# vikasdimaniya/video-fingerprinting

Measured on AMD Instinct MI355X. Metric: 1080p frames/sec embed+detect, higher is better.
Workload: dtype f32

## Files before the change

### include/offmark_hip.h

```cpp
#ifndef OFFMARK_HIP_H
#define OFFMARK_HIP_H

#include <stddef.h>
#include <stdint.h>

#ifdef __cplusplus
extern "C" {
#endif

#define OFMK_ABI_VERSION 6

#define OFMK_OK            0
#define OFMK_E_ARG        -1
#define OFMK_E_WORKSPACE  -2
#define OFMK_E_HIP        -3

int ofmk_version(void);
const char *ofmk_last_error(void);

typedef struct ofmk_timing ofmk_timing;
typedef struct ofmk_opts {
    uint32_t flags;
    uint32_t xcds;
    ofmk_timing *timing;
} ofmk_opts;
#define OFMK_F_SEPARATE_DETECT 1u
#define OFMK_F_LINEAR_TILES 2u
#define OFMK_F_XCD_TILES 4u
#define OFMK_XCD_TILES_MIN_BYTES 1194393600ull
#define OFMK_F_PARTIAL_COUNTS 8u
size_t ofmk_workspace_bytes(int frames_in_flight, int H, int W);

int ofmk_embed_rgb8(const uint8_t *in, uint8_t *out, int n, int H, int W,
                    const uint8_t *wm, int n_wm, const int32_t *wm_row, double alpha,
                    int chunk_frames, void *workspace, size_t workspace_bytes, void *stream,
                    const ofmk_opts *opts);

int ofmk_detect_rgb8(const uint8_t *in, int n, int H, int W, int L, double alpha,
                     int32_t *counts, uint8_t *bits,
                     int chunk_frames, void *workspace, size_t workspace_bytes, void *stream,
                     const ofmk_opts *opts);

int ofmk_detect_soft_rgb8(const uint8_t *in, int n, int H, int W, int L, double alpha, long long *soft,
                          int chunk_frames, void *workspace, size_t workspace_bytes, void *stream,
                          const ofmk_opts *opts);

int ofmk_embed_detect_rgb8(const uint8_t *in, uint8_t *out, int n, int H, int W,
                           const uint8_t *wm, int n_wm, const int32_t *wm_row, double alpha,
                           int L, int32_t *counts, uint8_t *bits,
                           int chunk_frames, void *workspace, size_t workspace_bytes, void *stream,
                           const ofmk_opts *opts);

int ofmk_svd_embed_rgb8(const uint8_t *in, uint8_t *out, int n, int H, int W,
                        const uint8_t *wm, int n_wm, const int32_t *wm_row, const double *scales, int blk, void *stream,
                        const ofmk_opts *opts);
int ofmk_svd_detect_rgb8(const uint8_t *in, int n, int H, int W, int L, const double *scales, int blk,
                         int32_t *counts, uint8_t *bits, void *stream, const ofmk_opts *opts);
int ofmk_svd_embed_detect_rgb8(const uint8_t *in, uint8_t *out, int n, int H, int W,
                               const uint8_t *wm, int n_wm, const int32_t *wm_row, const double *scales, int blk,
                               int L, int32_t *counts, uint8_t *bits, void *stream, const ofmk_opts *opts);
int ofmk_svd_detect_soft_rgb8(const uint8_t *in, int n, int H, int W, int L, const double *scales, int blk,
                              long long *soft, void *stream, const ofmk_opts *opts);
int ofmk_svd_sync_scores_rgb8(const uint8_t *in, int n, int H, int W, const double *scales, int blk, long long *scores,
// ... 118 lines not shown
int ofmk_halve_rgb8(const uint8_t *in, int n, int h, int w, uint8_t *out, void *stream, const ofmk_opts *opts);

int ofmk_signature_rgb8(const uint8_t *in, int n, int h, int w, uint8_t *sig, void *stream, const ofmk_opts *opts);
int ofmk_signature_distances(const uint8_t *a, int m, const uint8_t *b, int N, int32_t *dist, void *stream, const ofmk_opts *opts);
int ofmk_align_residuals_rgb8(const uint8_t *lib, int N, const uint8_t *leak, int m, int h, int w, int H, int W, const int32_t *first,
                              int span, const ofmk_affine *geom, long long *res, void *stream, const ofmk_opts *opts);

int ofmk_payloads_from_counts(const int32_t *counts, int n, int L, int n_bits, const int32_t *perm,
                              uint8_t *payload, void *stream, const ofmk_opts *opts);
int ofmk_svd_count_tiles(int H, int W, int blk);
int ofmk_payloads_from_partial_counts(const int32_t *partials, int tiles, int n, int L, int n_bits, const int32_t *perm,
                                      uint8_t *payload, int32_t *counts, void *stream, const ofmk_opts *opts);

int ofmk_encode_yuv32f(float *yuv, int n, int H, int W,
                       const uint8_t *wm, int n_wm, const int32_t *wm_row, double alpha,
                       int chunk_frames, void *workspace, size_t workspace_bytes, void *stream,
                       const ofmk_opts *opts);
int ofmk_decode_yuv32f(const float *yuv, int n, int H, int W, int L, double alpha,
                       int32_t *counts, uint8_t *bits,
                       int chunk_frames, void *workspace, size_t workspace_bytes, void *stream,
                       const ofmk_opts *opts);

int ofmk_debug_planes(const void *frame, int src_is_yuv32f, int H, int W, double alpha,
                      const uint8_t *wm,
                      float *y_dc, double *lum_mask, double *tex_mask, double *step,
                      float *c21_pre, float *c21_post,
                      void *workspace, size_t workspace_bytes, void *stream, const ofmk_opts *opts);

int ofmk_stage_analyze_rgb8(const uint8_t *in, int n, int H, int W,
                            void *workspace, size_t workspace_bytes, void *stream, const ofmk_opts *opts);
int ofmk_stage_mark_rgb8(const uint8_t *in, uint8_t *out, int n, int H, int W,
                         const uint8_t *wm, double alpha, int fused,
                         void *workspace, size_t workspace_bytes, void *stream, const ofmk_opts *opts);

int ofmk_hbm_copy(const void *src, void *dst, size_t bytes, void *stream);
int ofmk_hbm_read(const void *src, size_t bytes, void *sink, void *stream);

int ofmk_probe_xcc(int32_t *xcc_of_workgroup, int n_workgroups, void *stream, const ofmk_opts *opts);

#define OFMK_TIMING_KINDS 7
int ofmk_timing_create(int max_launches, unsigned kind_mask, ofmk_timing **out);
int ofmk_timing_collect(ofmk_timing *t, double *ms_by_kind , int *launches_by_kind );
int ofmk_timing_durations(ofmk_timing *t, float *ms_per_launch, int *kind_per_launch , int cap);
void ofmk_timing_destroy(ofmk_timing *t);

#ifdef __cplusplus
}
#endif
#endif
```

### video-fingerprinting_amd/csrc/offmark_kernels.hip

```cpp
#include <hip/hip_runtime.h>
#include <hip/hip_ext.h>

#include <atomic>
#include <cstdint>
#include <cstdio>
#include <cstring>
#include <type_traits>

#include "../../include/offmark_hip.h"

#include "common.hiph"
#include "readout.hiph"
#include "dct_kernels.hiph"
#include "svd_kernels.hiph"
#include "svd8_kernels.hiph"
#include "misc_kernels.hiph"
#include "planar_kernels.hiph"
#include "svd_planar_kernels.hiph"
#include "copies_kernels.hiph"
#include "planar_copies_kernels.hiph"
#include "resync_kernels.hiph"
#include "dct_resync_kernels.hiph"
#include "planar_resync_kernels.hiph"
#include "warp_kernels.hiph"
// ... 123 lines not shown

constexpr size_t kFixedBytes = 4096;

size_t tiles_per_frame(int H, int W) { return ((size_t)(H / 8) * (W / 8) + kThreads - 1) / kThreads; }

size_t per_frame_bytes(int H, int W) {
    const size_t nblk = (size_t)(H / 8) * (W / 8);
    return nblk * (kRec + 1) * sizeof(float) + 2 * tiles_per_frame(H, W) * 8;
}

int carve(void *ws, size_t bytes, int H, int W, int want_frames, Workspace &out) {
    if (!ws) return fail(OFMK_E_ARG, "workspace is null%s");
    if ((uintptr_t)ws % 256) return fail(OFMK_E_ARG, "workspace must be 256-byte aligned%s");
    const size_t per = per_frame_bytes(H, W);
    if (bytes < per + kFixedBytes) return fail(OFMK_E_WORKSPACE, "workspace smaller than ofmk_workspace_bytes(1, H, W)%s");
    size_t cap = (bytes - kFixedBytes) / per;
    if (want_frames > 0 && (size_t)want_frames < cap) cap = want_frames;
    if (cap > (size_t)kMaxChunk) cap = kMaxChunk;
    const size_t nblk = (size_t)(H / 8) * (W / 8);
    char *p = static_cast<char *>(ws);
    out.frames = (int)cap;
    out.tiles = (int)tiles_per_frame(H, W);
    out.plane = cap * nblk;
    out.rec = reinterpret_cast<float *>(p);
    p += align256(out.plane * kRec * sizeof(float));
    out.delta = reinterpret_cast<float *>(p);
    p += align256(out.plane * sizeof(float));
    out.ysum = reinterpret_cast<unsigned long long *>(p);
    p += align256(cap * out.tiles * 8);
    out.ysum2 = reinterpret_cast<unsigned long long *>(p);
    return OFMK_OK;
}

int check_opts(const ofmk_opts *o) {
    if (o && ((o->flags & ~(uint32_t)(OFMK_F_SEPARATE_DETECT | OFMK_F_LINEAR_TILES | OFMK_F_XCD_TILES | OFMK_F_PARTIAL_COUNTS)) || o->xcds > 64u))
        return fail(OFMK_E_ARG, "ofmk_opts: unknown flag bits or xcds > 64%s");
    if (o && (o->flags & OFMK_F_LINEAR_TILES) && (o->flags & OFMK_F_XCD_TILES))
        return fail(OFMK_E_ARG, "ofmk_opts: OFMK_F_LINEAR_TILES and OFMK_F_XCD_TILES exclude each other%s");
    return OFMK_OK;
}

int check_dims(int n, int H, int W) {
    if (n <= 0) return fail(OFMK_E_ARG, "n must be positive%s");
    if (H < 8 || W < 8) return fail(OFMK_E_ARG, "H and W must be at least 8%s");
    if ((long long)H * W >= (1LL << 28)) return fail(OFMK_E_ARG, "frame too large (H*W must be < 2^28)%s");
    return OFMK_OK;
}

int check_embed_args(const void *in, const void *out, int n, int H, int W, const uint8_t *wm, int n_wm) {
    int rc = check_dims(n, H, W);
    if (rc) return rc;
    if (!in || !out || !wm) return fail(OFMK_E_ARG, "null frame or watermark pointer%s");
    if (n_wm < 1) return fail(OFMK_E_ARG, "n_wm must be >= 1%s");
    return OFMK_OK;
}

int check_detect_args(const void *in, int n, int H, int W, int L, const int32_t *counts, const uint8_t *bits) {
    int rc = check_dims(n, H, W);
    if (rc) return rc;
    if (!in) return fail(OFMK_E_ARG, "null frame pointer%s");
    if (L < 1) return fail(OFMK_E_ARG, "payload length L must be >= 1%s");
    if (!counts && !bits) return fail(OFMK_E_ARG, "both outputs (counts, bits) are null%s");
    return OFMK_OK;
}

int check_soft_args(const void *in, int n, int H, int W, int L, const long long *soft) {
    if (int rc = check_dims(n, H, W)) return rc;
    if (!in || !soft) return fail(OFMK_E_ARG, "null pointer%s");
    if (L < 1) return fail(OFMK_E_ARG, "payload length L must be >= 1%s");
    return OFMK_OK;
}

Geom make_geom(int H, int W, const Workspace &ws, int frames = 0, int xcds = 0) {
    Geom g;
    g.frames = frames;
    g.xcds = xcds;
    g.W = W;
    g.wb = W / 8;
// ... 46 lines not shown
    with_bool(aligned_rows(frames, W, src == SRC_RGB8 ? 1 : 4), [&](auto al) {
        constexpr bool AL = decltype(al)::value;
        if (src == SRC_RGB8) OFMK_TIMED_LAUNCH(timing, (analyze_kernel<SRC_RGB8, AL>), grid, dim3(kThreads), kAnalyzeLdsCap, s, frames, g, ws.rec, ws.ysum, zero_counts, L);
        else OFMK_TIMED_LAUNCH(timing, (analyze_kernel<SRC_YUV32F, AL>), grid, dim3(kThreads), 0, s, frames, g, ws.rec, ws.ysum, zero_counts, L);
    });
    HIP_TRY(hipGetLastError());
    return OFMK_OK;
}

int launch_finalize(FinArgs a, int n, const Ctx &cx) {
    const int per_wg = kThreads * kFinItems;
    const dim3 grid((unsigned)((a.N + per_wg - 1) / per_wg), (unsigned)n);
    ScopedTiming timing(KIND_FINALIZE, cx);
    with_bool(a.delta || a.soft || a.y_dc || a.lum || a.tex || a.step || a.c21_pre || a.c21_post, [&](auto full) {
        OFMK_TIMED_LAUNCH(timing, finalize_kernel<decltype(full)::value>, grid, dim3(kThreads), 0, cx.s, a);
    });
    HIP_TRY(hipGetLastError());
    return OFMK_OK;
}

MarkArgs mark_args(const Workspace &ws, int H, int W, const uint8_t *wm, int n_wm, const int32_t *wm_row, double alpha) {
    MarkArgs m;
    m.rec = ws.rec;
    m.ysum = ws.ysum;
    m.wm = wm;
    m.wm_row = wm_row;
    m.n_wm = n_wm;
    m.N = (int)((long long)H * W / 64);
    m.alpha = alpha;
    return m;
}

int launch_mark_rgb8(const uint8_t *in, uint8_t *out, int n, int H, int W, const uint8_t *wm, int n_wm, const int32_t *wm_row,
                     double alpha, const Workspace &ws, bool fused, const Ctx &cx) {
    hipStream_t s = cx.s;
    const int xc = tile_xcds(cx, (size_t)n * H * W * 3);
    const Geom g = make_geom(H, W, ws, n, xc);
    const dim3 grid = xcd_grid(g.nblk, n, xc);
    const MarkArgs m = mark_args(ws, H, W, wm, n_wm, wm_row, alpha);
    {
        ScopedTiming timing(fused ? KIND_MARK_FUSED : KIND_MARK, cx);
        with_bool(aligned_rows(in, W, 1) && aligned_rows(out, W, 1), [&](auto al) {
            constexpr bool AL = decltype(al)::value;
            if (fused) OFMK_TIMED_LAUNCH(timing, (mark_rgb8_kernel<AL, true>), grid, dim3(kThreads), 0, s, in, out, g, m, ws.rec, ws.ysum2);
            else if (xc > 1) OFMK_TIMED_LAUNCH(timing, (mark_rgb8_kernel<AL, false, true>), grid, dim3(kThreads), 0, s, in, out, g, m, ws.rec, ws.ysum2);
            else OFMK_TIMED_LAUNCH(timing, (mark_rgb8_kernel<AL, false>), grid, dim3(kThreads), 0, s, in, out, g, m, ws.rec, ws.ysum2);
        });
    }
    HIP_TRY(hipGetLastError());
    if (in != out && (H % 8 || W % 8)) {
        launch_copy_fringe(in, out, n, H, W, (H / 8) * 8, (W / 8) * 8, s);
        HIP_TRY(hipGetLastError());
    }
    return OFMK_OK;
}

struct RecView {
    const float *rec;
    const unsigned long long *ysum;
    size_t plane;
    int tiles;
};
RecView input_records(const Workspace &ws) { return {ws.rec, ws.ysum, ws.plane, ws.tiles}; }
RecView marked_records(const Workspace &ws) { return {ws.rec, ws.ysum2, ws.plane, ws.tiles}; }

FinArgs fin_base(const RecView &v, int H, int W, double alpha) {
    FinArgs a;
    memset(&a, 0, sizeof(a));
    a.rec = v.rec;
    a.plane = v.plane;
    a.ysum = v.ysum;
    a.tiles = v.tiles;
    a.nblk = (H / 8) * (W / 8);
    a.N = (int)((long long)H * W / 64);
    a.L = 1;
    a.n_wm = 1;
    a.alpha = alpha;
// ... 572 lines not shown
    HIP_TRY(launch_zero(soft, (size_t)copies * n * L * sizeof(long long), cx.s));
    const bool on = a.scales[1] > 0.f;
    if (blk == 4) return fused(a, on ? soft : nullptr);
    return launch_svd8_copies(out, frame_bytes, copies, n, H, W, wm_rows, a, [&](uint8_t *out_q, const SvdArgs &b) {
        if (int rc = single(out_q, b)) return rc;
        if (!on) return (int)OFMK_OK;
        const size_t q = (size_t)(out_q - out) / ((size_t)n * frame_bytes);
        SvdArgs bs = b;
        bs.counts = reinterpret_cast<int32_t *>(soft + q * n * L);
        bs.bits = nullptr;
        bs.partial = 0;
        return soft_of(out_q, bs);
    });
}

enum FrameKind { FRAMES_RGB8, FRAMES_YUV32F, FRAMES_YUV420 };
struct FrameFmt {
    FrameKind kind;
    int layout;
    int H, W;
    size_t frame_bytes;
};
FrameFmt rgb8_frames(int H, int W) { return {FRAMES_RGB8, 0, H, W, (size_t)H * W * 3}; }
FrameFmt yuv32f_frames(int H, int W) { return {FRAMES_YUV32F, 0, H, W, (size_t)H * W * 3 * sizeof(float)}; }
FrameFmt yuv420_frames(int layout, int H, int W) { return {FRAMES_YUV420, layout, H, W, (size_t)H * W * 3 / 2}; }

int analyze_frames(const FrameFmt &f, const uint8_t *frames, int n, const Workspace &ws, const Ctx &cx, int32_t *zero_counts = nullptr,
                   int L = 0) {
    if (f.kind == FRAMES_YUV420) return launch_analyze_yuv420(frames, f.layout, n, f.H, f.W, ws, cx, zero_counts, L);
    return launch_analyze(frames, f.kind == FRAMES_RGB8 ? SRC_RGB8 : SRC_YUV32F, n, f.H, f.W, ws, cx, zero_counts, L);
}

int mark_frames(const FrameFmt &f, const uint8_t *in, uint8_t *out, int n, const uint8_t *wm, int n_wm, const int32_t *wm_row,
                double alpha, const Workspace &ws, bool fused, const Ctx &cx) {
    if (f.kind == FRAMES_RGB8) return launch_mark_rgb8(in, out, n, f.H, f.W, wm, n_wm, wm_row, alpha, ws, fused, cx);
    if (f.kind == FRAMES_YUV420) return launch_mark_yuv420(in, out, f.layout, n, f.H, f.W, wm, n_wm, wm_row, alpha, ws, fused, cx);
    if (fused || in != out) return fail(OFMK_E_ARG, "internal: float32 frames are marked in place, without verify%s");
    return launch_mark_yuv32f(reinterpret_cast<float *>(out), n, f.H, f.W, wm, n_wm, wm_row, alpha, ws, cx);
}

int mark_copies(const FrameFmt &f, const uint8_t *in, uint8_t *out, int copies, int n, int f0, int cf, const uint8_t *wm, int n_wm,
                const int32_t *wm_rows, double alpha, const Workspace &ws, const Ctx &cx) {
    if (f.kind == FRAMES_RGB8) return launch_mark_copies_rgb8(in, out, copies, n, f0, cf, f.H, f.W, wm, n_wm, wm_rows, alpha, ws, cx);
    if (f.kind == FRAMES_YUV420)
        return launch_mark_copies_yuv420(in, out, f.layout, copies, n, f0, cf, f.H, f.W, wm, n_wm, wm_rows, alpha, ws, cx);
    return fail(OFMK_E_ARG, "internal: no copies kernel for float32 frames%s");
}

int mark_verify_copies(const FrameFmt &f, const uint8_t *in, uint8_t *out, int copies, int n, int f0, int cf, const uint8_t *wm,
                       int n_wm, const int32_t *wm_rows, double alpha, int L, int32_t *zero_counts, const CopiesWorkspace &ws,
                       const Ctx &cx) {
    CopyRecs v;
    v.rec = ws.rec;
    v.ysum = ws.ysum;
    v.plane = ws.plane;
    v.rec_stride = (size_t)ws.base.frames * (f.H / 8) * (f.W / 8);
    v.ysum_stride = (size_t)ws.base.frames * ws.base.tiles;
    v.zero_counts = zero_counts ? zero_counts + (size_t)f0 * L : nullptr;
    v.L = L;
    if (f.kind == FRAMES_RGB8)
        return launch_mark_verify_copies_rgb8(in, out, copies, n, f0, cf, f.H, f.W, wm, n_wm, wm_rows, alpha, L, v, ws.base, cx);
    if (f.kind == FRAMES_YUV420)
        return launch_mark_verify_copies_yuv420(in, out, f.layout, copies, n, f0, cf, f.H, f.W, wm, n_wm, wm_rows, alpha, L, v, ws.base, cx);
    return fail(OFMK_E_ARG, "internal: no copies kernel for float32 frames%s");
}

int read_out(const RecView &v, const FrameFmt &f, size_t row, int cf, int L, double alpha, int32_t *counts, uint8_t *bits,
             long long *soft, const Ctx &cx) {
    FinArgs a = fin_base(v, f.H, f.W, alpha);
    a.L = L;
    if (counts || bits) {
        a.counts = counts ? counts + row * L : nullptr;
        a.bits = bits ? bits + row * a.N : nullptr;
        if (int rc = launch_finalize(a, cf, cx)) return rc;
    }
    if (!soft) return OFMK_OK;
    a.counts = nullptr;
    a.bits = nullptr;
    a.soft = soft + row * L;
    return launch_finalize(a, cf, cx);
}

int embed_chunk(const FrameFmt &f, const uint8_t *in, uint8_t *out, int f0, int cf, const uint8_t *wm, int n_wm, const int32_t *wm_row,
                double alpha, const Workspace &ws, bool verify, const Ctx &cx, int32_t *zero_counts = nullptr, int L = 0) {
    const size_t fo = (size_t)f0 * f.frame_bytes;
    if (int rc = analyze_frames(f, in + fo, cf, ws, cx, zero_counts ? zero_counts + (size_t)f0 * L : nullptr, L)) return rc;
    return mark_frames(f, in + fo, out + fo, cf, wm, n_wm, wm_row ? wm_row + f0 : nullptr, alpha, ws, verify, cx);
}

int detect_chunk(const FrameFmt &f, const uint8_t *in, int f0, int cf, int L, double alpha, int32_t *counts, uint8_t *bits,
                 long long *soft, const Workspace &ws, const Ctx &cx) {
    if (int rc = analyze_frames(f, in + (size_t)f0 * f.frame_bytes, cf, ws, cx, counts ? counts + (size_t)f0 * L : nullptr, L)) return rc;
    return read_out(input_records(ws), f, (size_t)f0, cf, L, alpha, counts, bits, soft, cx);
}

int embed_frames(const FrameFmt &f, const uint8_t *in, uint8_t *out, int n, const uint8_t *wm, int n_wm, const int32_t *wm_row,
                 double alpha, int chunk_frames, void *workspace, size_t workspace_bytes, void *stream, const ofmk_opts *opts) {
    Workspace ws;
    if (int rc = carve(workspace, workspace_bytes, f.H, f.W, chunk_frames, ws)) return rc;
    const Ctx cx = make_ctx(stream, opts);
    return for_chunks(n, ws.frames, [&](int f0, int cf) { return embed_chunk(f, in, out, f0, cf, wm, n_wm, wm_row, alpha, ws, false, cx); });
}

int detect_frames(const FrameFmt &f, const uint8_t *in, int n, int L, double alpha, int32_t *counts, uint8_t *bits, long long *soft,
                  int chunk_frames, void *workspace, size_t workspace_bytes, void *stream, const ofmk_opts *opts) {
    Workspace ws;
    if (int rc = carve(workspace, workspace_bytes, f.H, f.W, chunk_frames, ws)) return rc;
    const Ctx cx = make_ctx(stream, opts);
    if (soft) HIP_TRY(launch_zero(soft, (size_t)n * L * sizeof(long long), cx.s));
    return for_chunks(n, ws.frames, [&](int f0, int cf) { return detect_chunk(f, in, f0, cf, L, alpha, counts, bits, soft, ws, cx); });
}

int embed_detect_frames(const FrameFmt &f, const uint8_t *in, uint8_t *out, int n, const uint8_t *wm, int n_wm, const int32_t *wm_row,
                        double alpha, int L, int32_t *counts, uint8_t *bits, int chunk_frames, void *workspace, size_t workspace_bytes,
                        void *stream, const ofmk_opts *opts) {
    Workspace ws;
    if (int rc = carve(workspace, workspace_bytes, f.H, f.W, chunk_frames, ws)) return rc;
    const Ctx cx = make_ctx(stream, opts);
    return for_chunks(n, ws.frames, [&](int f0, int cf) {
        if (!(cx.flags & OFMK_F_SEPARATE_DETECT)) {
            if (int rc = embed_chunk(f, in, out, f0, cf, wm, n_wm, wm_row, alpha, ws, true, cx, counts, L)) return rc;
            return read_out(marked_records(ws), f, (size_t)f0, cf, L, alpha, counts, bits, nullptr, cx);
        }
        if (int rc = embed_chunk(f, in, out, f0, cf, wm, n_wm, wm_row, alpha, ws, false, cx)) return rc;
        return detect_chunk(f, out, f0, cf, L, alpha, counts, bits, nullptr, ws, cx);
    });
}

int embed_copies_frames(const FrameFmt &f, const uint8_t *in, uint8_t *out, int copies, int n, const uint8_t *wm, int n_wm,
                        const int32_t *wm_rows, double alpha, int chunk_frames, void *workspace, size_t workspace_bytes, void *stream,
                        const ofmk_opts *opts) {
    Workspace ws;
    if (int rc = carve(workspace, workspace_bytes, f.H, f.W, chunk_frames, ws)) return rc;
    const Ctx cx = make_ctx(stream, opts);
    int rc = for_chunks(n, ws.frames, [&](int f0, int cf) {
        if (int rc = analyze_frames(f, in + (size_t)f0 * f.frame_bytes, cf, ws, cx)) return rc;
        return mark_copies(f, in, out, copies, n, f0, cf, wm, n_wm, wm_rows, alpha, ws, cx);
    });
    if (rc) return rc;
    return launch_copy_fringe_copies(in, out, copies, n, f.H, f.W, cx.s);
}

int embed_detect_copies_frames(const FrameFmt &f, const uint8_t *in, uint8_t *out, int copies, int n, const uint8_t *wm, int n_wm,
                               const int32_t *wm_rows, double alpha, int L, int32_t *counts, uint8_t *bits, long long *soft,
                               int chunk_frames, void *workspace, size_t workspace_bytes, void *stream, const ofmk_opts *opts) {
    CopiesWorkspace ws;
    if (int rc = carve_copies(workspace, workspace_bytes, copies, f.H, f.W, chunk_frames, ws)) return rc;
    const Ctx cx = make_ctx(stream, opts);
    const bool hard = counts || bits;
    const int nblk = (f.H / 8) * (f.W / 8);
    const size_t N = (size_t)((long long)f.H * f.W / 64);
    if (soft) HIP_TRY(launch_zero(soft, (size_t)copies * n * L * sizeof(long long), cx.s));
    int rc = for_chunks(n, ws.base.frames, [&](int f0, int cf) {
        if (int rc = analyze_frames(f, in + (size_t)f0 * f.frame_bytes, cf, ws.base, cx)) return rc;
        if (!(cx.flags & OFMK_F_SEPARATE_DETECT)) {
// ... 363 lines not shown
    a.wm = wm;
    a.y_dc = y_dc;
    a.lum = lum_mask;
    a.tex = tex_mask;
    a.step = step;
    a.c21_pre = c21_pre;
    a.c21_post = wm ? c21_post : nullptr;
    return launch_finalize(a, 1, cx);
}

int ofmk_stage_analyze_rgb8(const uint8_t *in, int n, int H, int W, void *workspace, size_t workspace_bytes,
                            void *stream, const ofmk_opts *opts) {
    if (int orc = check_opts(opts)) return orc;
    int rc = check_dims(n, H, W);
    if (rc) return rc;
    if (!in) return fail(OFMK_E_ARG, "null frame pointer%s");
    Workspace ws;
    if ((rc = carve(workspace, workspace_bytes, H, W, n, ws))) return rc;
    if (ws.frames < n) return fail(OFMK_E_WORKSPACE, "stage call needs workspace for all n frames%s");
    return analyze_frames(rgb8_frames(H, W), in, n, ws, make_ctx(stream, opts));
}

int ofmk_stage_mark_rgb8(const uint8_t *in, uint8_t *out, int n, int H, int W, const uint8_t *wm, double alpha,
                         int fused, void *workspace, size_t workspace_bytes, void *stream, const ofmk_opts *opts) {
    if (int orc = check_opts(opts)) return orc;
    int rc = check_embed_args(in, out, n, H, W, wm, 1);
    if (rc) return rc;
    Workspace ws;
    if ((rc = carve(workspace, workspace_bytes, H, W, n, ws))) return rc;
    if (ws.frames < n) return fail(OFMK_E_WORKSPACE, "stage call needs workspace for all n frames%s");
    return mark_frames(rgb8_frames(H, W), in, out, n, wm, 1, nullptr, alpha, ws, fused != 0, make_ctx(stream, opts));
}

int ofmk_svd_embed_rgb8(const uint8_t *in, uint8_t *out, int n, int H, int W, const uint8_t *wm, int n_wm,
                        const int32_t *wm_row, const double *scales, int blk, void *stream, const ofmk_opts *opts) {
    if (int orc = check_opts(opts)) return orc;
    int rc = check_embed_args(in, out, n, H, W, wm, n_wm);
    if (rc) return rc;
    if ((rc = check_blk(blk))) return rc;
    SvdArgs a;
    if ((rc = make_svd_args(a, H, W, scales, false, wm, n_wm, wm_row, 1, nullptr, nullptr, nullptr))) return rc;
    return launch_svd_rgb8(in, out, n, H, W, SVD_EMBED, blk, a, make_ctx(stream, opts));
}

int ofmk_svd_detect_rgb8(const uint8_t *in, int n, int H, int W, int L, const double *scales, int blk, int32_t *counts, uint8_t *bits,
                         void *stream, const ofmk_opts *opts) {
    if (int orc = check_opts(opts)) return orc;
    int rc = check_detect_args(in, n, H, W, L, counts, bits);
    if (rc) return rc;
    if ((rc = check_blk(blk))) return rc;
    SvdArgs a;
    if ((rc = make_svd_args(a, H, W, scales, true, nullptr, 0, nullptr, L, counts, bits, opts))) return rc;
    if (!(a.scales[1] > 0.f)) return zero_svd_readout(n, H, W, blk, a, static_cast<hipStream_t>(stream));
    return launch_svd_rgb8(in, nullptr, n, H, W, SVD_DETECT, blk, a, make_ctx(stream, opts));
}

int ofmk_svd_detect_soft_rgb8(const uint8_t *in, int n, int H, int W, int L, const double *scales, int blk, long long *soft,
                              void *stream, const ofmk_opts *opts) {
    if (int orc = check_opts(opts)) return orc;
    int rc = check_soft_args(in, n, H, W, L, soft);
    if (rc) return rc;
    if ((rc = check_blk(blk))) return rc;
    return svd_detect_soft(n, H, W, L, scales, soft, stream, [&](const SvdArgs &a) {
        return launch_svd_rgb8(in, nullptr, n, H, W, SVD_DETECT_SOFT, blk, a, make_ctx(stream, opts));
    });
}
// ... 890 lines not shown
```

### video-fingerprinting_amd/offmark/_hip.py

```python
from __future__ import annotations

import ctypes as C
import os

_LIB_PATH = os.path.join(os.path.dirname(os.path.abspath(__file__)), "_lib", "liboffmark_hip.so")

ABI_VERSION = 6


class Opts(C.Structure):
    _fields_ = [("flags", C.c_uint32), ("xcds", C.c_uint32), ("timing", C.c_void_p)]
    _timing = None


F_SEPARATE_DETECT = 1
F_LINEAR_TILES = 2
F_XCD_TILES = 4
F_PARTIAL_COUNTS = 8
XCD_TILES_MIN_BYTES = 192 * 1080 * 1920 * 3
YUV_I420, YUV_NV12 = 0, 1
TIMING_KINDS = ("analyze", "finalize", "mark", "mark_fused", "svd", "planar_analyze", "planar_mark")

_vp, _i32, _f64, _sz, _u32 = C.c_void_p, C.c_int, C.c_double, C.c_size_t, C.c_uint
_op = C.POINTER(Opts)
_dp = C.POINTER(C.c_double)


class Warp(C.Structure):
    _fields_ = [("ay", C.c_int64), ("by", C.c_int64), ("ax", C.c_int64), ("bx", C.c_int64)]


_wp = C.POINTER(Warp)


class Affine(C.Structure):
    _fields_ = [("ayy", C.c_int64), ("ayx", C.c_int64), ("by", C.c_int64), ("axy", C.c_int64), ("axx", C.c_int64), ("bx", C.c_int64)]


_ap = C.POINTER(Affine)

SIGNATURES = {
    "ofmk_version": (_i32, []),
    "ofmk_last_error": (C.c_char_p, []),
    "ofmk_workspace_bytes": (_sz, [_i32, _i32, _i32]),
    "ofmk_embed_rgb8": (_i32, [_vp, _vp, _i32, _i32, _i32, _vp, _i32, _vp, _f64, _i32, _vp, _sz, _vp, _op]),
    "ofmk_detect_rgb8": (_i32, [_vp, _i32, _i32, _i32, _i32, _f64, _vp, _vp, _i32, _vp, _sz, _vp, _op]),
    "ofmk_detect_soft_rgb8": (_i32, [_vp, _i32, _i32, _i32, _i32, _f64, _vp, _i32, _vp, _sz, _vp, _op]),
    "ofmk_embed_detect_rgb8": (_i32, [_vp, _vp, _i32, _i32, _i32, _vp, _i32, _vp, _f64, _i32, _vp, _vp, _i32, _vp, _sz,
                                      _vp, _op]),
    "ofmk_encode_yuv32f": (_i32, [_vp, _i32, _i32, _i32, _vp, _i32, _vp, _f64, _i32, _vp, _sz, _vp, _op]),
    "ofmk_decode_yuv32f": (_i32, [_vp, _i32, _i32, _i32, _i32, _f64, _vp, _vp, _i32, _vp, _sz, _vp, _op]),
    "ofmk_debug_planes": (_i32, [_vp, _i32, _i32, _i32, _f64, _vp, _vp, _vp, _vp, _vp, _vp, _vp, _vp, _sz, _vp, _op]),
    "ofmk_stage_analyze_rgb8": (_i32, [_vp, _i32, _i32, _i32, _vp, _sz, _vp, _op]),
    "ofmk_stage_mark_rgb8": (_i32, [_vp, _vp, _i32, _i32, _i32, _vp, _f64, _i32, _vp, _sz, _vp, _op]),
    "ofmk_svd_embed_rgb8": (_i32, [_vp, _vp, _i32, _i32, _i32, _vp, _i32, _vp, _dp, _i32, _vp, _op]),
    "ofmk_svd_detect_rgb8": (_i32, [_vp, _i32, _i32, _i32, _i32, _dp, _i32, _vp, _vp, _vp, _op]),
    "ofmk_svd_detect_soft_rgb8": (_i32, [_vp, _i32, _i32, _i32, _i32, _dp, _i32, _vp, _vp, _op]),
    "ofmk_svd_sync_scores_rgb8": (_i32, [_vp, _i32, _i32, _i32, _dp, _i32, _vp, _vp, _op]),
    "ofmk_svd_detect_soft_window_rgb8": (_i32, [_vp, _i32, _i32, _i32, _i32, _i32, _i32, _i32, _i32, _dp, _i32, _vp, _vp, _op]),
    "ofmk_sync_workspace_bytes": (_sz, [_i32, _i32, _i32]),
    "ofmk_sync_scores_rgb8": (_i32, [_vp, _i32, _i32, _i32, _f64, _vp, _i32, _vp, _sz, _vp, _op]),
    "ofmk_detect_soft_window_rgb8": (_i32, [_vp, _i32, _i32, _i32, _i32, _i32, _i32, _i32, _i32, _f64, _vp, _i32, _vp, _sz, _vp, _op]),
    "ofmk_svd_embed_detect_rgb8": (_i32, [_vp, _vp, _i32, _i32, _i32, _vp, _i32, _vp, _dp, _i32, _i32, _vp, _vp, _vp, _op]),
    "ofmk_embed_copies_rgb8": (_i32, [_vp, _vp, _i32, _i32, _i32, _i32, _vp, _i32, _vp, _f64, _i32, _vp, _sz, _vp, _op]),
    "ofmk_svd_embed_copies_rgb8": (_i32, [_vp, _vp, _i32, _i32, _i32, _i32, _vp, _i32, _vp, _dp, _i32, _i32, _vp, _vp, _vp,
                                          _op]),
    "ofmk_copies_workspace_bytes": (_sz, [_i32, _i32, _i32, _i32]),
    "ofmk_embed_detect_copies_rgb8": (_i32, [_vp, _vp, _i32, _i32, _i32, _i32, _vp, _i32, _vp, _f64, _i32, _vp, _vp, _i32, _vp, _sz,
                                             _vp, _op]),
    "ofmk_embed_detect_copies_soft_rgb8": (_i32, [_vp, _vp, _i32, _i32, _i32, _i32, _vp, _i32, _vp, _f64, _i32, _vp, _vp, _vp, _i32, _vp,
                                                  _sz, _vp, _op]),
    "ofmk_svd_embed_copies_soft_rgb8": (_i32, [_vp, _vp, _i32, _i32, _i32, _i32, _vp, _i32, _vp, _dp, _i32, _i32, _vp, _vp, _vp, _vp,
                                               _op]),
    "ofmk_svd_encode_yuv32f": (_i32, [_vp, _i32, _i32, _i32, _vp, _i32, _vp, _dp, _i32, _vp, _op]),
    "ofmk_svd_decode_yuv32f": (_i32, [_vp, _i32, _i32, _i32, _dp, _i32, _vp, _vp, _op]),
    "ofmk_payloads_from_counts": (_i32, [_vp, _i32, _i32, _i32, _vp, _vp, _vp, _op]),
    "ofmk_svd_count_tiles": (_i32, [_i32, _i32, _i32]),
    "ofmk_payloads_from_partial_counts": (_i32, [_vp, _i32, _i32, _i32, _i32, _vp, _vp, _vp, _vp, _op]),
    "ofmk_embed_yuv420": (_i32, [_vp, _vp, _i32, _i32, _i32, _i32, _vp, _i32, _vp, _f64, _i32, _vp, _sz, _vp, _op]),
    "ofmk_detect_yuv420": (_i32, [_vp, _i32, _i32, _i32, _i32, _i32, _f64, _vp, _vp, _i32, _vp, _sz, _vp, _op]),
    "ofmk_detect_soft_yuv420": (_i32, [_vp, _i32, _i32, _i32, _i32, _i32, _f64, _vp, _i32, _vp, _sz, _vp, _op]),
    "ofmk_embed_detect_yuv420": (_i32, [_vp, _vp, _i32, _i32, _i32, _i32, _vp, _i32, _vp, _f64, _i32, _vp, _vp, _i32, _vp,
                                        _sz, _vp, _op]),
    "ofmk_svd_embed_yuv420": (_i32, [_vp, _vp, _i32, _i32, _i32, _i32, _vp, _i32, _vp, _dp, _i32, _vp, _op]),
    "ofmk_svd_detect_yuv420": (_i32, [_vp, _i32, _i32, _i32, _i32, _i32, _dp, _i32, _vp, _vp, _vp, _op]),
    "ofmk_svd_detect_soft_yuv420": (_i32, [_vp, _i32, _i32, _i32, _i32, _i32, _dp, _i32, _vp, _vp, _op]),
    "ofmk_svd_embed_detect_yuv420": (_i32, [_vp, _vp, _i32, _i32, _i32, _i32, _vp, _i32, _vp, _dp, _i32, _i32, _vp, _vp, _vp,
# ... 154 lines not shown
```

Before: 282,500.

## Compute readout bits in fused mark kernel and count from per-wave masks

The fused mark kernel now computes each block's readout bit and a 'settled' flag, then stores them as per-wave ballot masks in the spare delta workspace. A new readout kernel counts bits from these masks, so the finalize pass no longer has to reread the full three-plane record array for every block. Blocks that are not settled (too close to the decision threshold) presumably fall back to the exact computation. This costs extra work and register pressure in the mark kernel, and it only applies when counts are requested, no bits are requested, and L is a power of two up to 64.

```diff
diff --git a/include/offmark_hip.h b/include/offmark_hip.h
--- a/include/offmark_hip.h
+++ b/include/offmark_hip.h
@@ -29,6 +29,7 @@
 #define OFMK_F_XCD_TILES 4u
 #define OFMK_XCD_TILES_MIN_BYTES 1194393600ull
 #define OFMK_F_PARTIAL_COUNTS 8u
+#define OFMK_F_PLAIN_READOUT 16u
 size_t ofmk_workspace_bytes(int frames_in_flight, int H, int W);
 
 int ofmk_embed_rgb8(const uint8_t *in, uint8_t *out, int n, int H, int W,
@@ -213,6 +214,12 @@
 int ofmk_stage_mark_rgb8(const uint8_t *in, uint8_t *out, int n, int H, int W,
                          const uint8_t *wm, double alpha, int fused,
                          void *workspace, size_t workspace_bytes, void *stream, const ofmk_opts *opts);
+int ofmk_stage_mark_masks_rgb8(const uint8_t *in, uint8_t *out, int n, int H, int W,
+                               const uint8_t *wm, double alpha, double delta,
+                               void *workspace, size_t workspace_bytes, void *stream, const ofmk_opts *opts);
+int ofmk_stage_readout_masks_rgb8(int n, int H, int W, int L, double alpha, double delta,
+                                  int32_t *counts, int32_t *stats,
+                                  void *workspace, size_t workspace_bytes, void *stream, const ofmk_opts *opts);
 
 int ofmk_hbm_copy(const void *src, void *dst, size_t bytes, void *stream);
 int ofmk_hbm_read(const void *src, size_t bytes, void *sink, void *stream);
diff --git a/video-fingerprinting_amd/csrc/dct_finalize_body.inc b/video-fingerprinting_amd/csrc/dct_finalize_body.inc
--- /dev/null
+++ b/video-fingerprinting_amd/csrc/dct_finalize_body.inc
@@ -0,0 +1,55 @@
+    __shared__ int hist[kHistMax];
+    __shared__ FrameLum s_lum;
+    const int t = threadIdx.x;
+    const int f = blockIdx.y;
+    const int c0 = tile_x * (kThreads * kFinItems) + t;
+    const bool use_hist = (p.counts != nullptr || (FULL && p.soft != nullptr)) && p.L <= kHistMax;
+    const bool pow2 = (p.L & (p.L - 1)) == 0;
+    if (use_hist)
+        for (int k = t; k < p.L; k += kThreads) hist[k] = 0;
+    float a00[kFinItems], tcode[kFinItems], c21[kFinItems];
+#pragma unroll
+    for (int i = 0; i < kFinItems; ++i) {
+        const int c = c0 + i * kThreads;
+        const float *r = p.rec + (size_t)f * p.nblk + (c < p.nblk ? c : p.nblk - 1);
+        a00[i] = r[0]; tcode[i] = r[p.plane]; c21[i] = r[2 * p.plane];
+    }
+    frame_lum_to_lds(p.ysum, f, p.tiles, p.nblk, &s_lum);
+    __syncthreads();
+    const FrameLum fl = s_lum;
+    const FastLum fq = make_fast_lum(fl, p.alpha);
+    const bool by_ballot = !FULL && p.counts != nullptr && pow2 && p.L <= 64;
+    unsigned long long own_mask = 0;
+    if (by_ballot)
+        for (int j = (int)(t & 63) & (p.L - 1); j < 64; j += p.L) own_mask |= 1ull << j;
+    unsigned own = 0;
+#pragma unroll
+    for (int i = 0; i < kFinItems; ++i) {
+        const int c = c0 + i * kThreads;
+        int bit = 0;
+        if constexpr (FULL) {
+            if (c < p.nblk) finalize_block<FULL>(p, f, c, fl, use_hist, hist, a00[i], tcode[i], c21[i], bit);
+        } else if (c < p.nblk) {
+            bit = readout_bit_fast(a00[i], tcode[i], c21[i], fl, fq, p.alpha);
+            if (p.bits) p.bits[(size_t)f * p.N + c] = (uint8_t)bit;
+        }
+        if (c >= p.nblk && c < p.N && p.bits) p.bits[(size_t)f * p.N + c] = 0;
+        if (by_ballot) {
+            const unsigned long long hit = __ballot(bit != 0) & own_mask;
+            own += __popc((unsigned)hit) + __popc((unsigned)(hit >> 32));
+        } else if (p.counts) {
+            count_bit(p, f, c, bit, pow2, use_hist, hist);
+        }
+    }
+    if (by_ballot && (int)(t & 63) < p.L && own) {
+        if (use_hist) atomicAdd(&hist[t & (p.L - 1)], (int)own);
+        else atomicAdd(&p.counts[(size_t)f * p.L + (t & (p.L - 1))], (int)own);
+    }
+    if (use_hist) {
+        __syncthreads();
+        for (int k = t; k < p.L; k += kThreads) {
+            const int v = hist[k];
+            if (FULL && v && p.soft) atomicAdd(reinterpret_cast<unsigned long long *>(&p.soft[(size_t)f * p.L + k]), (unsigned long long)(long long)v);
+            else if (v) atomicAdd(&p.counts[(size_t)f * p.L + k], v);
+        }
+    }
diff --git a/video-fingerprinting_amd/csrc/dct_mark_rgb8_body.inc b/video-fingerprinting_amd/csrc/dct_mark_rgb8_body.inc
--- /dev/null
+++ b/video-fingerprinting_amd/csrc/dct_mark_rgb8_body.inc
@@ -0,0 +1,40 @@
+    __shared__ FrameLum s_lum;
+    __shared__ long long s_part[kThreads / 64];
+    const int tiles = tiles_of(g.nblk);
+    int f, bx;
+    if (!xcd_tile(g.xcds, tiles, g.frames, f, bx)) return;
+    const int c = bx * kThreads + threadIdx.x;
+    const bool valid = c < g.nblk;
+    const int cc = valid ? c : g.nblk - 1;
+    int bi, bj;
+    divmod_small(cc, g.wb, g.inv_wb, bi, bj);
+    const size_t off = (size_t)f * g.frame_stride + ((size_t)bi * 8 * g.W + (size_t)bj * 8) * 3;
+    const int pitch = g.W * 3;
+    Px8 raw[8];
+#pragma unroll
+    for (int r = 0; r < 8; ++r) raw[r] = load_px8<ALIGNED>(in + off + (size_t)r * pitch);
+#pragma unroll
+    for (int r = 0; r < 8; ++r) forget(raw[r]);
+    frame_lum_to_lds(m.ysum, f, tiles, g.nblk, &s_lum);
+    __syncthreads();
+    if (!FUSED && !valid) return;
+    float R[8][8], u1[4];
+    float d;
+    {
+        const float *r = m.rec + (size_t)f * g.nblk + cc;
+        const int row = wm_row_of(m.wm_row, f, m.n_wm);
+        d = mark_delta(r[0], r[g.plane], r[2 * g.plane], s_lum, m.alpha, m.wm[(size_t)row * m.N + cc]);
+    }
+    mark_rows<ALIGNED, FUSED, HOLD>(raw, d, valid, out + off, pitch, R, u1);
+    if constexpr (FUSED) {
+        const BlockFeat ft = block_features(R, u1);
+        if constexpr (MASKS) {
+            const FrameLum fl = s_lum;
+            const SettledBit sb = readout_bit_settled(ft.a00, ft.tex, ft.c21, fl, make_fast_lum(fl, m.alpha), delta);
+            WaveMasks wmk;
+            wmk.settled = __ballot(!valid || sb.settled);
+            wmk.bits = __ballot(valid && sb.bit != 0);
+            if ((threadIdx.x & 63) == 0) summary[((size_t)f * tiles + bx) * kWavesPerTile + (threadIdx.x >> 6)] = wmk;
+        }
+        emit_block(ft, valid, f, c, bx, tiles, g, rec_out, ysum_out, s_part);
+    }
diff --git a/video-fingerprinting_amd/csrc/offmark_kernels.hip b/video-fingerprinting_amd/csrc/offmark_kernels.hip
--- a/video-fingerprinting_amd/csrc/offmark_kernels.hip
+++ b/video-fingerprinting_amd/csrc/offmark_kernels.hip
@@ -179,8 +179,13 @@
     return OFMK_OK;
 }
 
+WaveMasks *masks_of(const Workspace &ws) { return reinterpret_cast<WaveMasks *>(ws.delta); }
+bool masks_fit(const Workspace &ws, int frames) {
+    return (size_t)frames * ws.tiles * kWavesPerTile * sizeof(WaveMasks) <= align256(ws.plane * sizeof(float));
+}
+
 int check_opts(const ofmk_opts *o) {
-    if (o && ((o->flags & ~(uint32_t)(OFMK_F_SEPARATE_DETECT | OFMK_F_LINEAR_TILES | OFMK_F_XCD_TILES | OFMK_F_PARTIAL_COUNTS)) || o->xcds > 64u))
+    if (o && ((o->flags & ~(uint32_t)(OFMK_F_SEPARATE_DETECT | OFMK_F_LINEAR_TILES | OFMK_F_XCD_TILES | OFMK_F_PARTIAL_COUNTS | OFMK_F_PLAIN_READOUT)) || o->xcds > 64u))
         return fail(OFMK_E_ARG, "ofmk_opts: unknown flag bits or xcds > 64%s");
     if (o && (o->flags & OFMK_F_LINEAR_TILES) && (o->flags & OFMK_F_XCD_TILES))
         return fail(OFMK_E_ARG, "ofmk_opts: OFMK_F_LINEAR_TILES and OFMK_F_XCD_TILES exclude each other%s");
@@ -191,6 +196,11 @@
     if (n <= 0) return fail(OFMK_E_ARG, "n must be positive%s");
     if (H < 8 || W < 8) return fail(OFMK_E_ARG, "H and W must be at least 8%s");
     if ((long long)H * W >= (1LL << 28)) return fail(OFMK_E_ARG, "frame too large (H*W must be < 2^28)%s");
+    return OFMK_OK;
+}
+
+int check_delta(double delta) {
+    if (!(delta >= 0.0) || !(delta <= 255.0)) return fail(OFMK_E_ARG, "delta must lie in [0, 255]%s");
     return OFMK_OK;
 }
 
@@ -303,7 +313,7 @@
 }
 
 int launch_mark_rgb8(const uint8_t *in, uint8_t *out, int n, int H, int W, const uint8_t *wm, int n_wm, const int32_t *wm_row,
-                     double alpha, const Workspace &ws, bool fused, const Ctx &cx) {
+                     double alpha, const Workspace &ws, bool fused, const Ctx &cx, bool masks = false, double delta = kReadoutDelta) {
     hipStream_t s = cx.s;
     const int xc = tile_xcds(cx, (size_t)n * H * W * 3);
     const Geom g = make_geom(H, W, ws, n, xc);
@@ -313,7 +323,8 @@
         ScopedTiming timing(fused ? KIND_MARK_FUSED : KIND_MARK, cx);
         with_bool(aligned_rows(in, W, 1) && aligned_rows(out, W, 1), [&](auto al) {
             constexpr bool AL = decltype(al)::value;
-            if (fused) OFMK_TIMED_LAUNCH(timing, (mark_rgb8_kernel<AL, true>), grid, dim3(kThreads), 0, s, in, out, g, m, ws.rec, ws.ysum2);
+            if (fused && masks) OFMK_TIMED_LAUNCH(timing, (mark_masks_rgb8_kernel<AL>), grid, dim3(kThreads), 0, s, in, out, g, m, ws.rec, ws.ysum2, masks_of(ws), delta);
+            else if (fused) OFMK_TIMED_LAUNCH(timing, (mark_rgb8_kernel<AL, true>), grid, dim3(kThreads), 0, s, in, out, g, m, ws.rec, ws.ysum2);
             else if (xc > 1) OFMK_TIMED_LAUNCH(timing, (mark_rgb8_kernel<AL, false, true>), grid, dim3(kThreads), 0, s, in, out, g, m, ws.rec, ws.ysum2);
             else OFMK_TIMED_LAUNCH(timing, (mark_rgb8_kernel<AL, false>), grid, dim3(kThreads), 0, s, in, out, g, m, ws.rec, ws.ysum2);
         });
@@ -952,8 +963,9 @@
 }
 
 int mark_frames(const FrameFmt &f, const uint8_t *in, uint8_t *out, int n, const uint8_t *wm, int n_wm, const int32_t *wm_row,
-                double alpha, const Workspace &ws, bool fused, const Ctx &cx) {
-    if (f.kind == FRAMES_RGB8) return launch_mark_rgb8(in, out, n, f.H, f.W, wm, n_wm, wm_row, alpha, ws, fused, cx);
+                double alpha, const Workspace &ws, bool fused, const Ctx &cx, bool masks = false) {
+    if (f.kind == FRAMES_RGB8) return launch_mark_rgb8(in, out, n, f.H, f.W, wm, n_wm, wm_row, alpha, ws, fused, cx, masks);
+    if (masks) return fail(OFMK_E_ARG, "internal: only the fused RGB8 mark kernel leaves read-out masks%s");
     if (f.kind == FRAMES_YUV420) return launch_mark_yuv420(in, out, f.layout, n, f.H, f.W, wm, n_wm, wm_row, alpha, ws, fused, cx);
     if (fused || in != out) return fail(OFMK_E_ARG, "internal: float32 frames are marked in place, without verify%s");
     return launch_mark_yuv32f(reinterpret_cast<float *>(out), n, f.H, f.W, wm, n_wm, wm_row, alpha, ws, cx);
@@ -986,9 +998,22 @@
 }
 
 int read_out(const RecView &v, const FrameFmt &f, size_t row, int cf, int L, double alpha, int32_t *counts, uint8_t *bits,
-             long long *soft, const Ctx &cx) {
+             long long *soft, const Ctx &cx, const MaskArgs *masks = nullptr) {
     FinArgs a = fin_base(v, f.H, f.W, alpha);
     a.L = L;
+    if (masks) {
+        if (!counts || bits || soft) return fail(OFMK_E_ARG, "internal: the read-out by masks gives counts only%s");
+        a.counts = counts + row * L;
+        const int fin_tiles = (a.N + kThreads * kFinItems - 1) / (kThreads * kFinItems);
+        const int mask_wgs = (a.tiles * kWavesPerTile + kThreads - 1) / kThreads;
+        const int spare = 1536 / cf > 1 ? 1536 / cf : 1;
+        const int per_frame = mask_wgs > (spare < fin_tiles ? spare : fin_tiles) ? mask_wgs : (spare < fin_tiles ? spare : fin_tiles);
+        const dim3 grid((unsigned)per_frame, (unsigned)cf);
+        ScopedTiming timing(KIND_FINALIZE, cx);
+        OFMK_TIMED_LAUNCH(timing, readout_masks_kernel, grid, dim3(kThreads), 0, cx.s, a, *masks);
+        HIP_TRY(hipGetLastError());
+        return OFMK_OK;
+    }
     if (counts || bits) {
         a.counts = counts ? counts + row * L : nullptr;
         a.bits = bits ? bits + row * a.N : nullptr;
@@ -1001,11 +1026,21 @@
     return launch_finalize(a, cf, cx);
 }
 
+bool masks_usable(const FrameFmt &f, int cf, int L, double alpha, const int32_t *counts, const uint8_t *bits, const Workspace &ws,
+                  const Ctx &cx) {
+    return f.kind == FRAMES_RGB8 && counts && !bits && L <= 64 && (L & (L - 1)) == 0 && alpha >= 1e-3 && alpha <= 1e6 &&
+           !(cx.flags & OFMK_F_PLAIN_READOUT) && masks_fit(ws, cf);
+}
+MaskArgs marked_masks(const Workspace &ws, double delta = kReadoutDelta, int32_t *stats = nullptr) {
+    return {masks_of(ws), ws.ysum, delta, stats};
+}
+
 int embed_chunk(const FrameFmt &f, const uint8_t *in, uint8_t *out, int f0, int cf, const uint8_t *wm, int n_wm, const int32_t *wm_row,
-                double alpha, const Workspace &ws, bool verify, const Ctx &cx, int32_t *zero_counts = nullptr, int L = 0) {
+                double alpha, const Workspace &ws, bool verify, const Ctx &cx, int32_t *zero_counts = nullptr, int L = 0,
+                bool masks = false) {
     const size_t fo = (size_t)f0 * f.frame_bytes;
     if (int rc = analyze_frames(f, in + fo, cf, ws, cx, zero_counts ? zero_counts + (size_t)f0 * L : nullptr, L)) return rc;
-    return mark_frames(f, in + fo, out + fo, cf, wm, n_wm, wm_row ? wm_row + f0 : nullptr, alpha, ws, verify, cx);
+    return mark_frames(f, in + fo, out + fo, cf, wm, n_wm, wm_row ? wm_row + f0 : nullptr, alpha, ws, verify, cx, masks);
 }
 
 int detect_chunk(const FrameFmt &f, const uint8_t *in, int f0, int cf, int L, double alpha, int32_t *counts, uint8_t *bits,
@@ -1039,8 +1074,10 @@
     const Ctx cx = make_ctx(stream, opts);
     return for_chunks(n, ws.frames, [&](int f0, int cf) {
         if (!(cx.flags & OFMK_F_SEPARATE_DETECT)) {
-            if (int rc = embed_chunk(f, in, out, f0, cf, wm, n_wm, wm_row, alpha, ws, true, cx, counts, L)) return rc;
-            return read_out(marked_records(ws), f, (size_t)f0, cf, L, alpha, counts, bits, nullptr, cx);
+            const bool masks = masks_usable(f, cf, L, alpha, counts, bits, ws, cx);
+            if (int rc = embed_chunk(f, in, out, f0, cf, wm, n_wm, wm_row, alpha, ws, true, cx, counts, L, masks)) return rc;
+            const MaskArgs ma = marked_masks(ws);
+            return read_out(marked_records(ws), f, (size_t)f0, cf, L, alpha, counts, bits, nullptr, cx, masks ? &ma : nullptr);
         }
         if (int rc = embed_chunk(f, in, out, f0, cf, wm, n_wm, wm_row, alpha, ws, false, cx)) return rc;
         return detect_chunk(f, out, f0, cf, L, alpha, counts, bits, nullptr, ws, cx);
@@ -1470,6 +1507,39 @@
     return mark_frames(rgb8_frames(H, W), in, out, n, wm, 1, nullptr, alpha, ws, fused != 0, make_ctx(stream, opts));
 }
 
+int ofmk_stage_mark_masks_rgb8(const uint8_t *in, uint8_t *out, int n, int H, int W, const uint8_t *wm, double alpha, double delta,
+                               void *workspace, size_t workspace_bytes, void *stream, const ofmk_opts *opts) {
+    if (int orc = check_opts(opts)) return orc;
+    int rc = check_embed_args(in, out, n, H, W, wm, 1);
+    if (rc) return rc;
+    if ((rc = check_delta(delta))) return rc;
+    Workspace ws;
+    if ((rc = carve(workspace, workspace_bytes, H, W, n, ws))) return rc;
+    if (ws.frames < n) return fail(OFMK_E_WORKSPACE, "stage call needs workspace for all n frames%s");
+    if (!masks_fit(ws, n)) return fail(OFMK_E_WORKSPACE, "workspace has no room for the masks of n frames this small%s");
+    return launch_mark_rgb8(in, out, n, H, W, wm, 1, nullptr, alpha, ws, true, make_ctx(stream, opts), true, delta);
+}
+
+int ofmk_stage_readout_masks_rgb8(int n, int H, int W, int L, double alpha, double delta, int32_t *counts, int32_t *stats,
+                                  void *workspace, size_t workspace_bytes, void *stream, const ofmk_opts *opts) {
+    if (int orc = check_opts(opts)) return orc;
+    int rc = check_dims(n, H, W);
+    if (rc) return rc;
+    if (L < 1 || L > 64 || (L & (L - 1))) return fail(OFMK_E_ARG, "the read-out by masks needs L a power of two <= 64%s");
+    if (!(alpha >= 1e-3 && alpha <= 1e6)) return fail(OFMK_E_ARG, "the read-out by masks needs alpha in [1e-3, 1e6]%s");
+    if ((rc = check_delta(delta))) return rc;
+    if (!counts) return fail(OFMK_E_ARG, "null counts pointer%s");
+    Workspace ws;
+    if ((rc = carve(workspace, workspace_bytes, H, W, n, ws))) return rc;
+    if (ws.frames < n) return fail(OFMK_E_WORKSPACE, "stage call needs workspace for all n frames%s");
+    if (!masks_fit(ws, n)) return fail(OFMK_E_WORKSPACE, "workspace has no room for the masks of n frames this small%s");
+    const Ctx cx = make_ctx(stream, opts);
+    HIP_TRY(launch_zero(counts, (size_t)n * L * sizeof(int32_t), cx.s));
+    if (stats) HIP_TRY(launch_zero(stats, (size_t)n * 2 * sizeof(int32_t), cx.s));
+    const MaskArgs ma = marked_masks(ws, delta, stats);
+    return read_out(marked_records(ws), rgb8_frames(H, W), 0, n, L, alpha, counts, nullptr, nullptr, cx, &ma);
+}
+
 int ofmk_svd_embed_rgb8(const uint8_t *in, uint8_t *out, int n, int H, int W, const uint8_t *wm, int n_wm,
                         const int32_t *wm_row, const double *scales, int blk, void *stream, const ofmk_opts *opts) {
     if (int orc = check_opts(opts)) return orc;
diff --git a/video-fingerprinting_amd/offmark/_hip.py b/video-fingerprinting_amd/offmark/_hip.py
--- a/video-fingerprinting_amd/offmark/_hip.py
+++ b/video-fingerprinting_amd/offmark/_hip.py
@@ -17,6 +17,8 @@
 F_LINEAR_TILES = 2
 F_XCD_TILES = 4
 F_PARTIAL_COUNTS = 8
+F_PLAIN_READOUT = 16
+READOUT_DELTA = 0.125
 XCD_TILES_MIN_BYTES = 192 * 1080 * 1920 * 3
 YUV_I420, YUV_NV12 = 0, 1
 TIMING_KINDS = ("analyze", "finalize", "mark", "mark_fused", "svd", "planar_analyze", "planar_mark")
@@ -53,6 +55,8 @@
     "ofmk_debug_planes": (_i32, [_vp, _i32, _i32, _i32, _f64, _vp, _vp, _vp, _vp, _vp, _vp, _vp, _vp, _sz, _vp, _op]),
     "ofmk_stage_analyze_rgb8": (_i32, [_vp, _i32, _i32, _i32, _vp, _sz, _vp, _op]),
     "ofmk_stage_mark_rgb8": (_i32, [_vp, _vp, _i32, _i32, _i32, _vp, _f64, _i32, _vp, _sz, _vp, _op]),
+    "ofmk_stage_mark_masks_rgb8": (_i32, [_vp, _vp, _i32, _i32, _i32, _vp, _f64, _f64, _vp, _sz, _vp, _op]),
+    "ofmk_stage_readout_masks_rgb8": (_i32, [_i32, _i32, _i32, _i32, _f64, _f64, _vp, _vp, _vp, _sz, _vp, _op]),
     "ofmk_svd_embed_rgb8": (_i32, [_vp, _vp, _i32, _i32, _i32, _vp, _i32, _vp, _dp, _i32, _vp, _op]),
     "ofmk_svd_detect_rgb8": (_i32, [_vp, _i32, _i32, _i32, _i32, _dp, _i32, _vp, _vp, _vp, _op]),
     "ofmk_svd_detect_soft_rgb8": (_i32, [_vp, _i32, _i32, _i32, _i32, _dp, _i32, _vp, _vp, _op]),
```

Measured after the change: 284,100, median of 3. Within noise of the previous version (+0.6%).
